# getanteon/alaz

Measured on AMD Instinct MI355X. Metric: L7 edge-events/s ingested->scored service-map, higher is better.
Workload: dtype u64; 1 GPU; C3 device-resident replay: 10000 pods / 5000 services / 1000000 edges, 10000000 HTTP l7 events per window already in HBM, 2-layer SAGE + MLP score, partitioned K1 (variant 0, 8-byte records, 512 partitions); 2-batch HBM ring (value excludes PCIe: see end_to_end with --full); events_per_window=10000000, layers=2, windows_in_flight=1, parallelism=1 GPU

## Files before the change

### alaz_amd/csrc/servicegraph.hip

```cpp
#include <hip/hip_runtime.h>
#include <hip/hip_ext.h>

#include <algorithm>
#include <cmath>
#include <cstdio>
#include <cstring>
#include <chrono>
#include <condition_variable>
#include <thread>
#include <mutex>
#include <string>
#include <unordered_map>
#include <vector>

#include <dlfcn.h>

#include "join_host.hpp"
#include "sg_plan.hpp"
#include "sg_kernels.h"
#include "sg_sel.h"
#include "sg_trend.h"
#include "sg_node_trend.h"
#include "sg_rank.h"
#include "shard_seq.hpp"
// ... 367 lines not shown
    for (u32 k = 0; k < l; k++) n += 2 * (size_t)(k == 0 ? SG_F_IN : SG_F_HID) * SG_F_HID + SG_F_HID;
    return n;
}

void launch_halo_lists(sg_engine* e, hipStream_t s, u32* req, u32 capp) {
    if (e->plan.k6_one_wg) {
        if (e->d.ncap <= K6_FLAGS_LDS) hipLaunchKernelGGL(k6_halo_build_padded<true>, dim3(1), dim3(1024), 0, s, e->d, req, capp);
        else hipLaunchKernelGGL(k6_halo_build_padded<false>, dim3(1), dim3(1024), 0, s, e->d, req, capp);
        return;
    }
    hipLaunchKernelGGL(k6_halo_lists, dim3(((size_t)e->d.ncap + 1023) / 1024), dim3(1024), 0, s, e->d, req, capp, ++e->k6_epoch, 1u);
}
int do_close(sg_engine* e, hipStream_t s, const u32* d_union, const u32* d_union_n, u32 ob_mode = 1, u32 stride = 0, u32 gworld = 0, bool fuse_in = false) {
    int rc = sync_tables(e, s);
    if (rc) return rc;
    Dev dloc = e->d;
    if (dloc.warm && (size_t)e->cur < e->note_seen.size()) {
        volatile u64* note = e->h_note[e->cur];
        const u64 seq = note[0];
        if (seq != e->note_seen[e->cur]) {
            e->note_seen[e->cur] = seq;
            const u64 v = note[1];
            const u32 cold = (u32)(v & 0xFFu); const bool obip = (v & 0x100ull) != 0;
            e->cold_streak = cold == 2 ? e->cold_streak + 1 : 0;
            e->obip_streak = (cold == 1 && obip) ? e->obip_streak + 1 : 0;
            if (e->cold_streak >= 3) { e->plain_left = 32; e->cold_streak = 0; }
            if (e->obip_streak >= 4) { e->plain_left = 64; e->obip_streak = 0; }
        }
    }
    if (dloc.warm && e->plain_left) { e->plain_left--; dloc.warm = 0; }
    if ((size_t)e->cur < e->plain_slot.size()) e->plain_slot[e->cur] = e->d.warm && !dloc.warm;
    const Dev& d = dloc;
    bool warm_try = d.warm && e->warm_on;
    const u32 wt = warm_try ? 1u : 0u;
    {
        Timed tp(e, s, 2);
        if (ob_mode == 1) hipLaunchKernelGGL(kc_prepare, dim3(1), dim3(1024), 0, s, d, (u64)e->n_known, (u64)e->n_labels_decl, e->d_ob_list, (const u32*)e->d_ob_n, e->plan.ob_list_cap, 1u, (const u32*)nullptr, 0u, 0u, wt);
        else if (ob_mode == 0) hipLaunchKernelGGL(kc_prepare, dim3(1), dim3(1024), 0, s, d, (u64)e->n_known, (u64)e->n_labels_decl, const_cast<u32*>(d_union), d_union_n, e->plan.ob_list_cap, 0u, (const u32*)nullptr, 0u, 0u, wt);
        else hipLaunchKernelGGL(kc_prepare, dim3(1), dim3(1024), 0, s, d, (u64)e->n_known, (u64)e->n_labels_decl, e->d_ob_list, (const u32*)e->d_ob_n, e->plan.ob_list_cap, 2u, d_union, stride, gworld, wt);
    }
    if (d.variant == 0) {
        const bool tk = ((e->timing >> 7) & 1u) && e->closes % e->timing_stride == 0;
        hipEvent_t ta = tk ? get_event(e) : nullptr, tb = tk ? get_event(e) : nullptr;
        Dev db = d; db.batch_state = e->window_events_in == 0 ? 2u : 0u;
        db.kept_compact = d.warm;
        const dim3 grid(d.narrow ? d.npb : d.np), block(e->plan.k1b_threads);
        if (d.warm && warm_try) {
            hipExtLaunchKernelGGL(e->fn.k1b_try, grid, block, (uint32_t)e->plan.k1b_lds, s, ta, tb, 0u, db);
            if (tk) { TimingRec r; r.a = ta; r.b = tb; r.kernel = 7; e->trecs.push_back(r); ta = get_event(e); tb = get_event(e); }
        }
        hipExtLaunchKernelGGL(d.warm ? e->fn.k1b_cold : e->fn.k1b, grid, block, (uint32_t)e->plan.k1b_lds, s, ta, tb, 0u, db);
        if (tk) { TimingRec r; r.a = ta; r.b = tb; r.kernel = 7; e->trecs.push_back(r); }
    }
    {
        Timed t(e, s, 2);
        Dev dk = d;
        dk.kept_compact = d.warm;
        if (d.warm) {
            dk.rowptr = d.k_rowptr; dk.col = d.k_col; dk.csr_from = d.k_from; dk.acc_csr = d.k_acc; dk.max_edges = (u64)d.npb * d.pcap;
            dk.st_sum = e->scr_sum[e->cur]; dk.st_max = e->scr_max[e->cur]; dk.row_mu = e->scr_mu[e->cur]; dk.row_sd = e->scr_mu[e->cur] + d.ncap + 1;
        }
        if (d.variant == 1) {
            const u32 ntiles = e->plan.ecap / K2_TILE;
            hipLaunchKernelGGL(k2_edge_count, dim3(ntiles), dim3(256), 0, s, d);
            hipLaunchKernelGGL(k2_scan_tiles, dim3(1), dim3(1024), 0, s, d, ntiles);
            hipLaunchKernelGGL(k2_edge_compact, dim3(ntiles), dim3(256), 0, s, d);
        }
        if (d.dh_g) hipLaunchKernelGGL(k2_deg_hist, dim3(d.dh_g), dim3(K2_DH_THREADS), ((size_t)d.ncap + 1) * sizeof(u32), s, dk);
        const size_t rpr = d.dh_g ? K2_RP_ROWS_DH : K2_RP_ROWS;
        hipLaunchKernelGGL(e->fn.k2_rowptr, dim3(((size_t)d.ncap + rpr) / rpr), dim3(1024), 0, s, dk, ++e->rp_epoch);
        if (d.variant == 1) hipLaunchKernelGGL(k2_scatter_table, dim3(grid_for(e->cfg.max_edges, 256)), dim3(256), 0, s, d);
        else hipLaunchKernelGGL(k2_scatter_parts, dim3(d.npb), dim3(256), 0, s, dk);
        hipLaunchKernelGGL(k2_rowsort_gather, dim3(std::max(2, std::min(4096, 2 * K2_LONG_WGS + grid_for(d.ncap, 8)))), dim3(256), 2 * (size_t)d.k2_sortw * sizeof(u32), s, dk);
        if (d.warm) {
            const unsigned kg = (unsigned)(((u64)d.npb * d.pcap + KW_CH - 1) / KW_CH) + KW_CAPW;
            hipLaunchKernelGGL(kw_compact, dim3(kg), dim3(KW_THREADS), (size_t)KW_ROWS * 5 * sizeof(u64), s, d, ++e->kw_epoch, dk.st_sum, dk.st_max, (u64)(e->closes + 1), e->slots.size() > 1 ? 1u : 0u);
        }
    }
    {
        Timed t3(e, s, 8);
        const u32 fin = d.warm ? (u32)std::min<u64>(64, ((u64)d.ncap + 255) / 256) : 1u;
        if (fuse_in && e->plan.k3_fuse_allowed) {
            const u32 finp = d.warm ? (fin + 3) / 4 : 1u;
            hipLaunchKernelGGL(k3_in_part, dim3(e->plan.k3_ranges * e->plan.k3_slices + finp), dim3(1024), e->plan.k3in_lds, s, d, e->plan.k3_slices, finp);
            e->in_fused_slices = e->plan.k3_slices;
        } else {
            hipLaunchKernelGGL(k3_in_part, dim3(e->plan.k3_ranges * e->plan.k3_slices), dim3(1024), e->plan.k3in_lds, s, d, e->plan.k3_slices, 0u);
            hipLaunchKernelGGL(k3_in_reduce, dim3(grid_for((u64)d.ncap * 6, 256, 1024) + fin), dim3(256), 0, s, d, e->plan.k3_slices, fin);
            e->in_fused_slices = 0;
        }
    }
    HIP_TRY(e, hipGetLastError());
    e->closed = true;
    e->window_events_in = 0;
    e->closes++;
    return SG_OK;
}

int do_features(sg_engine* e, hipStream_t s) {
    const Dev& d = e->d;
    Timed t(e, s, 3);
    const int nbn = grid_for(d.ncap, 128), nbe = grid_for(e->cfg.max_edges, 256, 4096);
    hipLaunchKernelGGL(k3_node_features, dim3(nbn + nbe), dim3(256), 0, s, d, (u32)nbn, e->in_fused_slices);
    e->in_fused_slices = 0;
    HIP_TRY(e, hipGetLastError());
    return SG_OK;
}

int note_w_read(sg_engine* e, hipStream_t s) {
    for (auto& r : e->w_readers) if (r.first == s) { HIP_TRY(e, hipEventRecord(r.second, s)); return SG_OK; }
    for (size_t i = 0; i < e->w_readers.size();) {
        if (hipEventQuery(e->w_readers[i].second) == hipSuccess) { hipEventDestroy(e->w_readers[i].second); e->w_readers[i] = e->w_readers.back(); e->w_readers.pop_back(); }
        else i++;
    }
    hipEvent_t v = nullptr;
    HIP_TRY(e, hipEventCreateWithFlags(&v, hipEventDisableTiming));
    e->w_readers.emplace_back(s, v);
    HIP_TRY(e, hipEventRecord(v, s));
    return SG_OK;
}

int do_layer(sg_engine* e, u32 l, hipStream_t s, bool fuse_proj) {
    const Dev& d = e->d;
    if (!e->have_w) { e->err = "sg_load_weights not called"; return SG_ESTATE; }
    const float* Wl = e->d_W + layer_offset(l);
    const float* Wh = e->d_W + layer_offset(e->cfg.layers);
    const int grid = grid_for(d.ncap, 16);
    const bool pj = fuse_proj && l + 1 == e->cfg.layers && d.world == 1;
    Timed t(e, s, 4);
    const bool split = e->plan.k4_split;
    const int wide = l != 0;
    const float* hin = wide ? d.h[l] : d.x0;
    if (split) hipLaunchKernelGGL(kK4Gather[wide], dim3(grid_for(d.ncap, K4G_ROWS, 4096 * 8 / K4G_ROWS)), dim3(K4G_ROWS * 64), 0, s, d, hin);
    hipLaunchKernelGGL(e->fn.k4_layer[wide][pj], dim3(grid), dim3(k4_threads(wide ? 64 : 32, pj, split)), 0, s, d, hin, d.h[l + 1], Wl, Wh);
    HIP_TRY(e, hipGetLastError());
    return fuse_proj ? SG_OK : note_w_read(e, s);
}

static_assert(sizeof(sg_edge_vanished) == 64 && sgplan::kTrendThreads == K8_THREADS && sgplan::kTrendMaxWgs <= K8_SCAN_THREADS,
              "plan_trend / plan_vanished size the launches of sg_trend.h");
template <class Row>
TrendArgs baseline_args(const sg_engine* e, const sg_engine::Baseline<Row>& t) {
    const sg_trend_params& p = t.p;
    TrendArgs a{};
    a.ctr = e->d.ctr; a.ob_sorted = e->d.ob_sorted; a.max_obip = e->d.max_obip;
    a.cap = t.plan.entries;
    a.buf[0] = t.buf[0]; a.buf[1] = t.buf[1];
    a.th = t.th; a.blk = t.blk; a.ctl = t.ctl;
    a.w = t.w + 1; a.warmup = p.warmup; a.ttl = p.ttl;
    a.alpha = std::ldexp(1.0, -(int)p.shift); a.lat_floor = (double)p.lat_floor_ns; a.err_floor = (double)p.err_floor;
    return a;
}
template <class Row, class F>
int enqueue_baseline(sg_engine* e, sg_engine::Baseline<Row>& t, hipStream_t s, F launch) {
    if (t.pending) HIP_TRY(e, hipStreamWaitEvent(s, t.ev, 0));
    launch();
    HIP_TRY(e, hipGetLastError());
    HIP_TRY(e, hipEventRecord(t.ev, s));
    t.pending = true;
    t.w++;
    return SG_OK;
}
int launch_trend(sg_engine* e, hipStream_t s) {
    sg_engine::Baseline<sg_edge_trend>& t = e->trend;
    TrendArgs a = baseline_args(e, t);
    a.rows = e->d.rows; a.max_edges = e->cfg.max_edges; a.out = t.rows[e->cur];
    sg_engine::Vanished& v = e->vanished;
    return enqueue_baseline(e, t, s, [&] {
        if (v.on) {
            VanArgs va{};
            va.out = v.rows[e->cur]; va.count = v.count[e->cur]; va.th = v.th; va.blk = v.blk;
            va.max_rows = v.plan.rows; va.silent = v.p.silent_windows; va.min_seen = v.p.min_seen;
            hipLaunchKernelGGL(k8_count_v, dim3(t.plan.wgs), dim3(K8_THREADS), 0, s, a, va);
            hipLaunchKernelGGL(k8_scan_v, dim3(1), dim3(K8_SCAN_THREADS), 0, s, a, t.plan.wgs, va);
            hipLaunchKernelGGL(k8_write_v, dim3(t.plan.wgs), dim3(K8_THREADS), 0, s, a, va);
            v.valid[e->cur] = 1;
        } else {
            hipLaunchKernelGGL(k8_count, dim3(t.plan.wgs), dim3(K8_THREADS), 0, s, a);
            hipLaunchKernelGGL(k8_scan, dim3(1), dim3(K8_SCAN_THREADS), 0, s, a, t.plan.wgs);
            hipLaunchKernelGGL(k8_write, dim3(t.plan.wgs), dim3(K8_THREADS), 0, s, a);
        }
    });
}
static_assert(sgplan::kNodesThreads == K9_THREADS && sgplan::kNodesChunk == K9_CHUNK && sgplan::kNodesRangeNodes == K9_IN_NR &&
              sgplan::kNodesMaxWgs == K9_MAX_WGS && sgplan::kNodesMaxWgs <= K9_SCAN_THREADS && sgplan::kNodesSideBytes == sizeof(K9Side),
              "plan_nodes sizes the launches of sg_nodes.h");
// ... 1844 lines not shown
```

### alaz_amd/csrc/sg_k3.h

```cpp
#pragma once

__device__ __forceinline__ void alive_mark(const Dev& d, u32 g, u32 G, u32 t) {
    const u64 n_all = d.ctr[C_ALIVE_N];
    if (n_all == 0) return;
    const u32 n = (u32)(n_all < d.alive_cap ? n_all : d.alive_cap);
    const u32 nk = (u32)d.ctr[C_N_KNOWN], nl = (u32)d.ctr[C_N_LABELS], nob = (u32)d.ctr[C_N_OBIP];
    for (u32 i = g * 1024 + t; i < n; i += G * 1024) {
        const u64 key = d.alive_keys[i];
        const u32 f = dense_of(d, (u32)(key >> 32), nk, nl, nob), to = dense_of(d, (u32)key, nk, nl, nob);
        bool ok = f != SG_NONE && to != SG_NONE;
        if (ok) {
            u32 lo = d.rowptr[f], hi = d.rowptr[f + 1];
            if ((u64)hi > d.max_edges) hi = (u32)d.max_edges;
            const u32 end = hi;
            while (lo < hi) { const u32 m = (lo + hi) >> 1; if (d.col[m] < to) lo = m + 1; else hi = m; }
            ok = lo < end && d.col[lo] == to;
            if (ok) {
                atomicAdd(&d.alive_csr[lo], 1u);
                atomicAdd(&d.st_sum[(size_t)f * SG_NODE_STAT_SUM_WORDS + ST_OUT_ALIVE], 1ull);
                atomicAdd(&d.st_sum[(size_t)to * SG_NODE_STAT_SUM_WORDS + ST_IN_ALIVE], 1ull);
            }
        }
        if (!ok) atomicAdd(&d.ctr[C_ALIVE_DROP], 1ull);
    }
}

__global__ __launch_bounds__(1024) void k3_in_part(Dev d, u32 S, u32 fin) {
    extern __shared__ __attribute__((aligned(16))) unsigned char smem[];
    const u32 E = (u32)d.ctr[C_N_EDGES], N = (u32)d.ctr[C_N_NODES];
    const u32 G = gridDim.x - fin, g = blockIdx.x, t = threadIdx.x;
    if (g >= G) {
        if (d.warm) kw_finish_rows(d, (g - G) * 1024 + t, fin * 1024);
        else if (g == gridDim.x - 1) k2_split_finish(d, t, 1024);
        return;
    }
    SG_STAMP(d, 3, 0);
    if (g == 0 && t == 0 && d.warm && !d.ctr[C_COLD] && d.ctr[C_DELTA_N]) {
        d.ctr[C_KEPT_E] += (u64)d.dc_rowptr[d.max_known + d.max_labels];
        d.ctr[C_KEPT_BUF] ^= 1ull;
    }
    alive_mark(d, g, G, t);
    const u32 r = g / S, sl = g % S, n0 = r * K3_IN_NR;
    if (n0 >= N) return;
    const u32 nr = N - n0 < K3_IN_NR ? N - n0 : K3_IN_NR;
    u64* acc = reinterpret_cast<u64*>(smem);
    for (u32 i = t; i < nr * 6; i += 1024) acc[i] = 0;
    __syncthreads();
    SG_STAMP(d, 3, 1);
    const u32 per = (E + S - 1) / S, p0 = sl * per < E ? sl * per : E, p1 = p0 + per < E ? p0 + per : E;
    constexpr int K3Q = 8;
    u32 nxt[K3Q];
#pragma unroll
    for (int q = 0; q < K3Q; q++) { const u32 p = p0 + t + q * 1024; nxt[q] = p < p1 ? d.col[p] - n0 : 0xFFFFFFFFu; }
    for (u32 pb = p0 + t; pb < p1; pb += 1024 * K3Q) {
        u32 to[K3Q];
        ulonglong2 x[K3Q], y[K3Q];
#pragma unroll
        for (int q = 0; q < K3Q; q++) {
            to[q] = nxt[q];
            if (to[q] < nr) { const ulonglong2* a = reinterpret_cast<const ulonglong2*>(d.acc_csr + (size_t)(pb + q * 1024) * 4); x[q] = a[0]; y[q] = a[1]; }
        }
#pragma unroll
        for (int q = 0; q < K3Q; q++) { const u32 p = pb + 1024 * K3Q + q * 1024; nxt[q] = p < p1 ? d.col[p] - n0 : 0xFFFFFFFFu; }
#pragma unroll
        for (int q = 0; q < K3Q; q++) if (to[q] < nr) {
            u64* o = acc + (size_t)to[q] * 6;
            atomicAdd(&o[0], 1ull); atomicAdd(&o[1], x[q].x & 0xFFFFFFFFull); if (x[q].x >> 32) atomicAdd(&o[2], x[q].x >> 32);
            atomicAdd(&o[3], x[q].y); atomicAdd(&o[4], y[q].y); atomicMax(&o[5], y[q].x);
        }
    }
    SG_STAMP(d, 3, 2);
    __syncthreads();
    SG_STAMP(d, 3, 3);
    u64* out = d.in_part + ((size_t)r * S + sl) * K3_IN_NR * 6;
    for (u32 i = t; i < nr * 6; i += 1024) out[i] = acc[i];
    SG_STAMP(d, 3, 4);
}
__global__ __launch_bounds__(256) void k3_in_reduce(Dev d, u32 S, u32 fin) {
    const u32 N = (u32)d.ctr[C_N_NODES];
    if (blockIdx.x >= gridDim.x - fin) {
        if (d.warm) kw_finish_rows(d, (blockIdx.x - (gridDim.x - fin)) * 256 + threadIdx.x, fin * 256);
        else if (blockIdx.x == gridDim.x - 1) k2_split_finish(d, threadIdx.x, 256);
        return;
    }
    const u32 GW = gridDim.x - fin;
    for (u64 i = (u64)blockIdx.x * 256 + threadIdx.x; i < (u64)N * 6; i += (u64)GW * 256) {
        const u32 v = (u32)(i / 6), k = (u32)(i % 6), r = v / K3_IN_NR;
        const u64* p = d.in_part + ((size_t)r * S * K3_IN_NR + (v - r * K3_IN_NR)) * 6 + k;
        const size_t st = (size_t)K3_IN_NR * 6;
        u64 a = 0;
        u32 sl = 0;
        if (k == 5) {
            for (; sl + 8 <= S; sl += 8) {
                u64 x[8];
#pragma unroll
                for (int q = 0; q < 8; q++) x[q] = p[(size_t)(sl + q) * st];
#pragma unroll
                for (int q = 0; q < 8; q++) a = x[q] > a ? x[q] : a;
            }
            for (; sl < S; sl++) { const u64 x = p[(size_t)sl * st]; a = x > a ? x : a; }
            d.st_max[(size_t)v * 2 + 1] = a;
        } else {
            for (; sl + 8 <= S; sl += 8) {
                u64 x[8];
#pragma unroll
                for (int q = 0; q < 8; q++) x[q] = p[(size_t)(sl + q) * st];
#pragma unroll
                for (int q = 0; q < 8; q++) a += x[q];
            }
            for (; sl < S; sl++) a += p[(size_t)sl * st];
            d.st_sum[(size_t)v * SG_NODE_STAT_SUM_WORDS + (k == 0 ? ST_IN_DEG : k == 1 ? ST_IN_CNT : k == 2 ? ST_IN_ERR : k == 3 ? ST_IN_SUM : ST_IN_SSQ)] = a;
        }
    }
}

__global__ __launch_bounds__(256) void k3_node_features(Dev d, u32 nb_nodes, u32 S_in) {
    if (blockIdx.x >= nb_nodes) {
        const u32 E = (u32)d.ctr[C_N_EDGES];
        for (u32 p = (blockIdx.x - nb_nodes) * 256 + threadIdx.x; p < E; p += (gridDim.x - nb_nodes) * 256) edge_features(d, p);
        return;
    }
    const u32 N = (u32)d.ctr[C_N_NODES], nk = (u32)d.ctr[C_N_KNOWN];
    const u32 side = threadIdx.x & 1u;
    for (u32 v0 = blockIdx.x * 128; v0 < N; v0 += nb_nodes * 128) {
        const u32 v = v0 + (threadIdx.x >> 1);
        const bool live = v < N;
        float a[7] = {0.0f, 0.0f, 0.0f, 0.0f, 0.0f, 0.0f, 0.0f};
        if (live) {
            u64* s = d.st_sum + (size_t)v * SG_NODE_STAT_SUM_WORDS;
            u64 dg, c, er, sm, sq, mx;
            if (S_in && side) {
                const u32 r = v / K3_IN_NR;
                const ulonglong2* p = reinterpret_cast<const ulonglong2*>(d.in_part + ((size_t)r * S_in * K3_IN_NR + (v - r * K3_IN_NR)) * 6);
                const size_t st = (size_t)K3_IN_NR * 3;
                dg = c = er = sm = sq = mx = 0;
                u32 sl = 0;
                for (; sl + 4 <= S_in; sl += 4) {
                    ulonglong2 x[4][3];
#pragma unroll
                    for (int q = 0; q < 4; q++) { x[q][0] = p[(size_t)(sl + q) * st]; x[q][1] = p[(size_t)(sl + q) * st + 1]; x[q][2] = p[(size_t)(sl + q) * st + 2]; }
#pragma unroll
                    for (int q = 0; q < 4; q++) { dg += x[q][0].x; c += x[q][0].y; er += x[q][1].x; sm += x[q][1].y; sq += x[q][2].x; mx = x[q][2].y > mx ? x[q][2].y : mx; }
                }
                for (; sl < S_in; sl++) {
                    const ulonglong2 a0 = p[(size_t)sl * st], a1 = p[(size_t)sl * st + 1], a2 = p[(size_t)sl * st + 2];
                    dg += a0.x; c += a0.y; er += a1.x; sm += a1.y; sq += a2.x; mx = a2.y > mx ? a2.y : mx;
                }
                s[ST_IN_DEG] = dg; s[ST_IN_CNT] = c; s[ST_IN_ERR] = er; s[ST_IN_SUM] = sm; s[ST_IN_SSQ] = sq; d.st_max[(size_t)v * 2 + 1] = mx;
            } else {
                dg = s[ST_OUT_DEG + side]; c = s[ST_OUT_CNT + side]; er = s[ST_OUT_ERR + side]; sm = s[ST_OUT_SUM + side]; sq = s[ST_OUT_SSQ + side];
                mx = d.st_max[(size_t)v * 2 + side];
            }
            a[0] = (float)log1p((double)dg);
            a[1] = (float)log1p((double)c);
            a[2] = (float)log1p(mean_us(sm, c) / 1000.0);
            a[3] = c ? (float)((double)er / (double)c) : 0.0f;
            a[4] = (float)log1p((double)mx / 1e6);
            a[5] = (float)log1p(std_us(sm, sq, c) / 1000.0);
            a[6] = (float)log1p((double)s[ST_OUT_ALIVE + side]);
        }
        float b[7];
#pragma unroll
        for (int k = 0; k < 7; k++) b[k] = __shfl_xor(a[k], 1, 64);
        if (!live) continue;
        float4* o = reinterpret_cast<float4*>(d.x0 + (size_t)v * SG_F_IN);
        if (side == 0) {
            const u32 kind = v < nk ? d.kind[v] : 0u;
            o[0] = make_float4(a[0], b[0], a[1], b[1]);
            o[1] = make_float4(a[2], b[2], a[3], b[3]);
            o[2] = make_float4(a[4], b[4], kind == SG_NODE_POD ? 1.0f : 0.0f, kind == SG_NODE_SERVICE ? 1.0f : 0.0f);
            o[3] = make_float4(kind == 0 ? 1.0f : 0.0f, a[5], b[5], 1.0f);
        } else {
            o[4] = make_float4(b[6], a[6], 0.0f, 0.0f);
#pragma unroll
            for (int q = 5; q < (int)SG_F_IN / 4; q++) o[q] = make_float4(0.0f, 0.0f, 0.0f, 0.0f);
        }
    }
    if (blockIdx.x == 0 && threadIdx.x == 0) {
        const u64 n = d.ctr[C_ALIVE_N];
        d.ctr[C_ALIVE_SEEN] = n;
        d.ctr[C_ALIVE_DROPPED] = d.ctr[C_ALIVE_DROP] + (n > d.alive_cap ? n - d.alive_cap : 0);
        d.ctr[C_ALIVE_N] = 0; d.ctr[C_ALIVE_DROP] = 0;
    }
}

__global__ __launch_bounds__(256) void k_reset_window(Dev d) {
    const u64 tid = (u64)blockIdx.x * 256 + threadIdx.x, nt = (u64)gridDim.x * 256;
    const u64 nc = (u64)d.ncap + 1;
    if (!d.dh_g) for (u64 i = tid; i < nc * SG_DEG_REP; i += nt) { d.deg[i * SG_DEG_STRIDE] = 0; if (d.warm) d.deg2[i * SG_DEG_STRIDE] = 0; }
    for (u64 i = tid; i < nc; i += nt) d.cursor[i] = 0;
    for (u64 i = tid; i < (u64)d.ncap * SG_NODE_STAT_SUM_WORDS; i += nt) d.st_sum[i] = 0;
    for (u64 i = tid; i < (u64)d.ncap * SG_NODE_STAT_MAX_WORDS; i += nt) d.st_max[i] = 0;
    for (u64 i = tid; i <= d.obmask; i += nt) d.obkeys[i] = 0;
    for (u64 i = tid; i < (u64)SG_MAX_K1_WGS * WS_WORDS; i += nt) d.wgstat[i] = (i % WS_WORDS) == WS_TMIN ? ~0ull : 0ull;
    if (tid == 0) { d.ctr[C_OVF_N] = 0; d.ctr[C_ALIVE_N] = 0; d.ctr[C_ALIVE_DROP] = 0; }
    if (d.variant == 1 && d.ctr[C_EDGES_FOUND] > d.max_edges) {
        for (u64 i = tid; i <= d.emask; i += nt) {
            d.ekeys[i] = SG_EKEY_EMPTY;
            ulonglong2* a = reinterpret_cast<ulonglong2*>(d.eacc + (size_t)i * 4);
            a[0] = make_ulonglong2(0, 0); a[1] = make_ulonglong2(0, 0);
            if (d.hist) { uint4* hs = reinterpret_cast<uint4*>(d.hist_src + (size_t)i * SG_HIST_BINS); const uint4 z = make_uint4(0, 0, 0, 0); hs[0] = z; hs[1] = z; hs[2] = z; hs[3] = z; }
        }
    }
}
```

### alaz_amd/csrc/sg_plan.hpp

```cpp
#pragma once
#include <algorithm>
#include <array>
#include <cmath>
#include <cstdint>
#include <cstdlib>
#include <cstring>
#include <optional>
#include <string>

#include "../../include/servicegraph.h"
#include "sg_sizes.h"

namespace sgplan {

typedef uint32_t u32;
typedef uint64_t u64;

constexpr size_t kLdsBytes = 160 * 1024;
constexpr int kStageSlots = 32;

inline u32 next_pow2(u64 v) { u64 p = 1; while (p < v) p <<= 1; return (u32)p; }
inline int grid_for(u64 items, int per_block, int cap = 2048) {
    u64 g = (items + per_block - 1) / per_block;
    return (int)std::max<u64>(1, std::min<u64>(g, (u64)cap));
}

struct DeviceFacts {
    int cus = 256;
    size_t lds_bytes = kLdsBytes;
};

struct Overrides {
    typedef std::optional<std::string> Knob;
    Knob ablate, np, ht, ct, nwg, nsub, split, warm, k1a, k1_narrow, k1_legacy, k1b_u, k1b_threads, k1b_pack, k1b_no_order,
         l2_global, l2_u32, dh_g, k3_slices, k3_no_fuse, k4_fused, k5_grid, k6_one_wg, dense_valu, copy_streams, stage_slots, arena;
};
struct KnobName { const char* name; Overrides::Knob Overrides::*field; };
constexpr KnobName kKnobs[] = {
    {"SG_ABLATE", &Overrides::ablate}, {"SG_NP", &Overrides::np}, {"SG_HT", &Overrides::ht}, {"SG_CT", &Overrides::ct},
    {"SG_NWG", &Overrides::nwg}, {"SG_NSUB", &Overrides::nsub}, {"SG_SPLIT", &Overrides::split}, {"SG_WARM", &Overrides::warm},
    {"SG_K1A", &Overrides::k1a}, {"SG_K1_NARROW", &Overrides::k1_narrow}, {"SG_K1_LEGACY", &Overrides::k1_legacy},
    {"SG_K1B_U", &Overrides::k1b_u}, {"SG_K1B_THREADS", &Overrides::k1b_threads}, {"SG_K1B_PACK", &Overrides::k1b_pack},
    {"SG_K1B_NO_ORDER", &Overrides::k1b_no_order}, {"SG_L2_GLOBAL", &Overrides::l2_global}, {"SG_L2_U32", &Overrides::l2_u32},
    {"SG_DH_G", &Overrides::dh_g}, {"SG_K3_SLICES", &Overrides::k3_slices}, {"SG_K3_NO_FUSE", &Overrides::k3_no_fuse},
    {"SG_K4_FUSED", &Overrides::k4_fused}, {"SG_K5_GRID", &Overrides::k5_grid}, {"SG_K6_ONE_WG", &Overrides::k6_one_wg},
    {"SG_DENSE_VALU", &Overrides::dense_valu}, {"SG_COPY_STREAMS", &Overrides::copy_streams}, {"SG_STAGE_SLOTS", &Overrides::stage_slots},
    {"SG_ARENA", &Overrides::arena},
};
#ifdef SG_DEV_KNOBS
inline Overrides from_env() {
    Overrides o;
    for (const KnobName& k : kKnobs) if (const char* v = std::getenv(k.name)) o.*k.field = std::string(v);
    return o;
}
#endif
inline int ival(const Overrides::Knob& k) { return std::atoi(k->c_str()); }
inline u64 uval(const Overrides::Knob& k) { return std::strtoull(k->c_str(), nullptr, 0); }

struct Plan {
    u32 variant = 0, narrow = 0, hist = 0, agg_slots = 3, nb = 0, np = 0, pb = 0, nwg = 256, k1b_split = 1, k1b_ht = 0, npb = 0, rb = 0,
        pcap = 0, sa = 0, sn = 0, sw = 0, punits = 0, ss = 0, pslots = 0, ovf_cap = 0, warm = 0;
    u32 k1b_threads = 1024, k1b_u = 4;
    bool k1b_pack = false;
    bool k1b_order = false;
    size_t k1b_lds = 0;
    u32 ecap = 0, obcap = 0, ob_list_cap = 0, ncap = 0, max_obip = 1, alive_cap = 0, hub_cap = 0, max_blocks = 0;
    u64 kept_edges = 0;
    u32 max_known = 0;
    u32 k3_ranges = 1, k3_slices = 8;
    size_t k3in_lds = 0;
    u32 k2_sortw = 0, dh_g = 0, dh_ppw = 0, dh_ns = 0;
    bool k4_split = false;
    u32 k5_grid = 0;
    bool k3_fuse_allowed = true;
    bool k6_one_wg = false;
    bool use_mfma = true;
    u32 cus = 1;
    int k1_grid = 0, n_copy = 1, n_stage = 16;
    bool arena_on = false;
    u32 n_slots = 1;
    u32 ablate = 0;
};

struct PassA {
    bool l2_u16 = false, k1a_team = false, l2_in_lds = false;
    u32 k1a_nsub = 2, k1a_teams = 2, k1a_nt = 1024, k1a_ct = 2048;
    size_t k1a_lds = 0;
};

inline int check_config(const sg_config& in, sg_config* out) {
    constexpr uint32_t kCfgMin = 88;
    if (in.struct_size < kCfgMin || in.struct_size > 4096) return SG_EINVAL;
    sg_config c; std::memset(&c, 0, sizeof c);
    std::memcpy(&c, &in, std::min<size_t>(in.struct_size, sizeof c));
    c.struct_size = (uint32_t)sizeof c;
    if (c.abi_version != SG_ABI_VERSION || c.layers < 1 || c.layers > SG_MAX_LAYERS || c.max_edges == 0 ||
        c.max_known_nodes == 0 || c.world == 0 || c.rank >= c.world || c.max_known_nodes > 0x3FFFFFFFu)
        return SG_EINVAL;
    if (c.max_batch == 0) c.max_batch = 1u << 20;
    if (c.max_ips == 0) c.max_ips = c.max_known_nodes;
    if (c.max_window_events == 0) c.max_window_events = c.max_batch;
    *out = c;
    return SG_OK;
}

inline int make_plan(const sg_config& cfg, const DeviceFacts& dev, const Overrides& ov, Plan* out, std::string* why) {
    sg_config chk;
    if (check_config(cfg, &chk) != SG_OK) { if (why) *why = "invalid config"; return SG_EINVAL; }
    Plan p;
    const size_t lds = dev.lds_bytes;
    if (ov.arena) p.arena_on = ival(ov.arena) != 0;
    p.k1_grid = std::min<int>(SG_MAX_K1_WGS, dev.cus * 8);
    p.cus = (u32)std::max(1, dev.cus);
    p.use_mfma = !(ov.dense_valu && (*ov.dense_valu)[0] == '1');
    p.max_known = cfg.max_known_nodes;

    const u64 ME = cfg.max_edges;
    p.ecap = next_pow2(std::max<u64>(2 * ME, K2_TILE));
    p.obcap = next_pow2(std::max<u64>(2 * (u64)cfg.max_outbound_ips, 64));
    p.ob_list_cap = next_pow2(std::max<u64>((u64)cfg.max_outbound_ips * std::max<u32>(cfg.world, 1), 64));
    p.max_obip = std::max<u32>(cfg.max_outbound_ips, 1);
    p.ncap = cfg.max_known_nodes + cfg.max_labels + p.max_obip;

    p.variant = cfg.k1_variant == 1 ? 1u : 0u;
    p.hist = (cfg.flags & SG_CFG_EDGE_HISTOGRAM) ? 1u : 0u;
    p.agg_slots = p.hist ? 5u : 3u;
    const u64 cn = (u64)cfg.max_known_nodes + cfg.max_labels + p.obcap;
    u32 nb = 12; while ((1ull << nb) < cn && nb < 31) nb++;
    bool narrow = p.variant == 0 && !p.hist && cfg.k1_variant != 2 && !ov.k1_legacy && nb <= 24;
    const bool small_window = ME < (1ull << 18) && cfg.max_window_events <= (2ull << 20);
    if (cfg.k1_variant == 0 && small_window && !ov.k1_narrow) narrow = false;
    u64 np = 0;
    if (narrow) {
        np = next_pow2(std::max<u64>((ME + 2699) / 2700, 256));
        u32 pbt = 0; while ((1ull << pbt) < np) pbt++;
        if (np > 2048 || 2 * nb - pbt > 31) narrow = false;
    }
    p.k1b_split = 1;
    if (narrow) {
        if (ME / np > 1150) { p.k1b_split = 2; p.k1b_ht = 2048; }
        else p.k1b_ht = ME / np > 550 ? 2048 : 1024;
        if (ov.split) { const int x = ival(ov.split); if (x == 1 || x == 2) { p.k1b_split = (u32)x; p.k1b_ht = ME / (np * x) > 1150 ? 4096 : (ME / (np * x) > 550 ? 2048 : 1024); } }
    } else {
        np = next_pow2(std::max<u64>((ME + 1249) / 1250, 256));
        if (np > 4096) np = 4096;
        if (cfg.k1_variant != 1 && ME > (u64)4096 * 1400) p.variant = 1;
        p.k1b_ht = ME / np > 600 ? 2048 : 1024;
        if (p.hist && p.k1b_ht == 2048) { p.k1b_ht = 1024; np = std::min<u64>(4096, np * 2); }
    }
    p.np = (u32)np; p.nwg = 256;
    if (ov.np) { const u64 x = uval(ov.np); if (x >= 64 && x <= (narrow ? 2048u : 4096u) && (x & (x - 1)) == 0) p.np = (u32)x; }
    if (ov.ht) { const u64 x = uval(ov.ht); if (x >= 256 && x <= (narrow ? 4096u : 2048u) && (x & (x - 1)) == 0) p.k1b_ht = (u32)x; }
    if (ov.nwg) { const u64 x = uval(ov.nwg); if (x >= 1 && x <= (u64)SG_MAX_K1_WGS) p.nwg = (u32)x; }
    p.pb = 0; while ((1u << p.pb) < p.np) p.pb++;
    if (narrow && 2 * nb - p.pb > 31) { p.np = (u32)np; p.pb = 0; while ((1u << p.pb) < p.np) p.pb++; }
    p.narrow = (narrow && p.variant == 0) ? 1u : 0u;
    if (!p.narrow) p.k1b_split = 1;
    p.warm = (p.narrow && !p.hist && !(cfg.flags & SG_CFG_NO_WARM) && ((cfg.flags & SG_CFG_WARM) || ME >= (1ull << 18))) ? 1u : 0u;
    if (ov.warm) p.warm = (ival(ov.warm) != 0 && p.narrow && !p.hist) ? 1u : 0u;
    p.npb = p.np * p.k1b_split;
    p.nb = nb; p.rb = 2 * nb - p.pb;
    p.pcap = p.narrow ? p.k1b_ht * 13 / 16 : p.k1b_ht * 3 / 4;
    const double m = (double)cfg.max_window_events / ((double)p.np * p.nwg);
    p.sa = std::min<u32>(24, std::max<u32>(8, (2 * 2048 / p.np + 6 + 1) & ~1u));
    if (p.narrow) {
        p.sn = ((u32)(2.0 * m + 8.0 * std::sqrt(m + 1.0) + 24.0) + 1u) & ~1u;
        p.sn = std::min<u32>(p.sn, (1u << 20) - 16);
        p.sw = std::min<u32>(64, std::max<u32>(8, p.sn / 8));
        p.punits = (p.sn + 2 * p.sw + 5 * p.sa + 15) / 16 * 16;
        p.sn = p.punits - 2 * p.sw - 5 * p.sa;
        p.ss = 0; p.pslots = 0;
    } else {
        p.ss = (u32)(2.0 * m + 8.0 * std::sqrt(m + 1.0) + 24.0);
        p.ss = (p.ss + p.agg_slots * p.sa + 7) / 8 * 8 - p.agg_slots * p.sa;
        p.ss = std::min<u32>(p.ss, (1u << 20) - 8);
        p.pslots = p.ss + p.agg_slots * p.sa;
    }
    p.ovf_cap = 1u << 16;
    p.k1b_threads = 1024u;
    if (p.variant == 0)
        p.k1b_lds = p.narrow ? ((size_t)p.k1b_ht * 36 + 8 + (size_t)p.k1b_ht / 4 + 12 + 15) / 16 * 16 : (size_t)p.k1b_ht * (8 + 32 + (p.hist ? 4 * SG_HIST_BINS : 0));
    if (p.narrow) p.k1b_u = 2 * p.k1b_lds > lds && m > 24.0 ? 8 : 4;
    if (ov.k1b_u) { if (ival(ov.k1b_u) == 8) p.k1b_u = 8; if (ival(ov.k1b_u) == 4) p.k1b_u = 4; }
    if (p.k1b_u == 8) p.warm = 0;
    p.k1b_pack = p.narrow && (u64)p.sn * p.nwg < 65536ull;
    if (ov.k1b_pack) { if (ival(ov.k1b_pack) == 0) p.k1b_pack = false; }
    if (ov.k1b_threads) { const u64 x = uval(ov.k1b_threads); if ((x == 256 && !p.narrow) || x == 512 || x == 1024) p.k1b_threads = (u32)x; }
    if (p.narrow && p.k1b_ht / p.k1b_threads > 4) p.k1b_threads = 1024u;
    p.k1b_order = p.narrow && !ov.k1b_no_order;
    p.max_blocks = p.variant == 0 ? (u32)std::min<u64>(1024, std::max<u64>(64, (u64)cfg.max_ips / 32)) : 2u;
    if (p.variant == 0) p.ecap = K2_TILE;
    p.alive_cap = cfg.max_alive ? cfg.max_alive : 65536u;
    p.kept_edges = p.warm ? std::max<u64>(ME, (u64)p.npb * p.pcap) : ME;
    p.hub_cap = (u32)std::min<u64>(p.kept_edges / 256 + 16, 1u << 24);

    p.k3_ranges = (p.ncap + K3_IN_NR - 1) / K3_IN_NR;
    p.k3_slices = (u32)std::min<u64>((u64)p.k3_ranges * K3_IN_SMAX <= p.cus ? K3_IN_SMAX : 32, std::max<u64>(8, ME / 8192));
    if (ov.k3_slices) { const u64 x = uval(ov.k3_slices); if (x >= 1 && x <= 256) p.k3_slices = (u32)x; }
    p.k3in_lds = (size_t)K3_IN_NR * 48;
    {
        const u64 bw = ((u64)p.ncap + 31) / 32;
        p.k2_sortw = bw <= K2_SORT_LDS ? K2_SORT_LDS : (u32)std::min<u64>(K2_SORT_LDS_MAX, (bw + 255) / 256 * 256);
    }
    {
        u32 g = std::min<u32>(K2_DH_GMAX, p.variant == 0 ? p.npb : 0u);
        if (ME < (1ull << 19)) g = 0;
        if (p.warm) g = 0;
        else if (ov.dh_g) { const u64 x = uval(ov.dh_g); g = (x >= 16 && x <= K2_DH_GMAX && (x & (x - 1)) == 0 && p.variant == 0 && x <= p.npb) ? (u32)x : 0u; }
        if (g >= 16 && (g & (g - 1)) == 0 && p.npb % g == 0 && ((size_t)p.ncap + 1) * sizeof(u32) <= 128u * 1024u && (u64)p.npb * p.pcap < (1ull << 32)) {
            p.dh_g = g; p.dh_ppw = p.npb / g; p.dh_ns = (p.ncap + 1 + 63u) & ~63u;
        }
    }
    p.ablate = ov.ablate ? (u32)std::strtoul(ov.ablate->c_str(), nullptr, 0) : 0u;
    p.k4_split = cfg.max_edges > (1u << 17);
    if (ov.k4_fused) p.k4_split = ival(ov.k4_fused) == 0;
    p.k5_grid = (u32)grid_for(cfg.max_edges, 32, 3 * (int)p.cus);
    if (ov.k5_grid) { const int x = ival(ov.k5_grid); if (x >= 1 && x <= 65535) p.k5_grid = (u32)std::min(grid_for(cfg.max_edges, 32, 65535), x); }
    p.k3_fuse_allowed = !ov.k3_no_fuse;
    p.k6_one_wg = (bool)ov.k6_one_wg;
    if (ov.copy_streams) p.n_copy = ival(ov.copy_streams) == 2 ? 2 : 1;
    if (ov.stage_slots) p.n_stage = std::min(kStageSlots, std::max(2, ival(ov.stage_slots)));
    p.n_slots = std::min<u32>(std::max<u32>(cfg.windows_in_flight, 1), 8);
    *out = p;
    return SG_OK;
}

inline bool plan_pass_a(const Plan& p, uint32_t l1_entries, size_t l2_bytes, const Overrides& ov, PassA* out) {
    PassA a;
    const size_t lds_cap = kLdsBytes;
    const size_t l1b = (size_t)l1_entries * 8, l2b = l2_bytes;
    const size_t stage_max = (size_t)K1A_NJ * K1A_THREADS * 16;
    if (p.narrow) {
        a.l2_u16 = p.max_known <= 16384 && !ov.l2_u32;
        const size_t l2lds = a.l2_u16 ? l2b / 2 : l2b;
        if (ov.nsub) { const int x = ival(ov.nsub); if (x == 1 || x == 2) a.k1a_nsub = (u32)x; }
        const bool want_tile = ov.k1a && *ov.k1a == "tile", force_team = ov.k1a && *ov.k1a == "team";
        const size_t fixed_tile = (size_t)p.np * 24 + 64 + (size_t)K1T_TS(a.k1a_nsub) * 8 + l1b;
        const int teams = 2, nt = 1024;
        const size_t stage_team = (size_t)K1A_NJ * nt * 16;
        const bool team_ok = (p.np == 256 || p.np == 512 || p.np == 1024) && (size_t)p.np * p.nwg * p.punits * 8 < ((size_t)1 << 31) && l1b <= stage_team;
        a.k1a_teams = (u32)teams; a.k1a_nt = (u32)nt;
        const size_t fixed_team = K1M_LDS_FIXED(p.np, teams, nt) + l1b;
        auto pick = [&](size_t fixed, u32 ct_min, size_t stage_cap, u32& ct, bool& in_lds) {
            ct = 0; in_lds = false;
            for (u32 c : {1024u, 512u, 256u, 128u}) if (c >= ct_min && (size_t)c * 40 + fixed + l2lds <= lds_cap && l1b + l2b <= stage_cap) { in_lds = true; ct = c; break; }
            if (!ct) for (u32 c : {1024u, 512u, 256u, 128u, 64u}) if (c >= ct_min && (size_t)c * 40 + fixed <= lds_cap) { ct = c; break; }
        };
        u32 ct = 0; bool in_lds = false;
        if (!want_tile && team_ok) { pick(fixed_team, force_team ? 64u : 256u, stage_team, ct, in_lds); a.k1a_team = ct != 0; }
        if (!ct) pick(fixed_tile, 64u, stage_max, ct, in_lds);
        const size_t fixed = a.k1a_team ? fixed_team : fixed_tile;
        a.l2_in_lds = in_lds;
        if (ov.l2_global) a.l2_in_lds = false;
        if (ov.ct) { const u32 x = (u32)std::strtoul(ov.ct->c_str(), nullptr, 0); if (x >= 64 && x <= 2048 && (x & (x - 1)) == 0 && (size_t)x * 40 + fixed + (a.l2_in_lds ? l2lds : 0) <= lds_cap) ct = x; }
        if (!ct || l1b > stage_max) return false;
        a.k1a_ct = ct;
        a.k1a_lds = (size_t)ct * 40 + fixed + (a.l2_in_lds ? l2lds : 0);
        *out = a;
        return true;
    }
    const size_t fixed = (size_t)p.np * 4 + 64 + l1b;
    const size_t slot = p.hist ? 72 : 40;
    u32 ct = 0;
    for (u32 c : {2048u, 1024u, 512u}) if ((size_t)c * slot + fixed + l2b <= lds_cap && l1b + l2b <= stage_max) { a.l2_in_lds = true; ct = c; break; }
    if (!ct) for (u32 c : {2048u, 1024u, 512u, 256u, 128u, 64u}) if ((size_t)c * slot + fixed <= lds_cap) { ct = c; break; }
    if (ov.ct) { const u32 x = (u32)std::strtoul(ov.ct->c_str(), nullptr, 0); if (x >= 64 && x <= 2048 && (x & (x - 1)) == 0 && (size_t)x * slot + fixed + (a.l2_in_lds ? l2b : 0) <= lds_cap) ct = x; }
    if (ov.l2_global) a.l2_in_lds = false;
    if (!ct || l1b > stage_max) return false;
    a.k1a_ct = ct;
    a.k1a_lds = (size_t)ct * slot + fixed + (a.l2_in_lds ? l2b : 0);
    *out = a;
    return true;
}

enum K1aFamily { K1A_GLOBAL = 0, K1A_WIDE = 1, K1A_TILE = 2, K1A_TEAM = 3 };
enum K1bFamily { K1B_NONE = 0, K1B_MERGE = 1, K1B_STREAM = 2 };
constexpr int kK1bWarmU = 2;
struct PassAKernel {
    int family = K1A_GLOBAL;
// ... 274 lines not shown
```

### alaz_amd/csrc/sg_sizes.h

```cpp
#pragma once

#define SG_MAX_K1_WGS 2048

#define K1A_THREADS 1024
#define K1A_NJ      6
#define K1T_THREADS 1024
#define K1T_CHUNK   4096u
#define K1T_TS(NSUB) (K1T_CHUNK * (NSUB))
#define K1M_LDS_FIXED(np, teams, nt) ((size_t)(np) * 4 * (2 + 4 * (teams)) + 128 + ((size_t)(nt) * 4 + 4) * 8)

#define K2_TILE 2048
#define K2_DH_GMAX 128
#define K2_SORT_LDS 4096
#define K2_SORT_LDS_MAX 16384

#define K3_IN_NR    3072
#define K3_IN_SMAX  48

#define KW_ROWS 512
```

Baseline: 23.03 billion events/s.

## Interleave node-to-range mapping in k3 in-degree partial reduction

Result: no change. 23.23 billion events/s (median of 6 runs) (+0.9%).

```diff
diff --git a/alaz_amd/csrc/servicegraph.hip b/alaz_amd/csrc/servicegraph.hip
--- a/alaz_amd/csrc/servicegraph.hip
+++ b/alaz_amd/csrc/servicegraph.hip
@@ -473,11 +473,11 @@
         const u32 fin = d.warm ? (u32)std::min<u64>(64, ((u64)d.ncap + 255) / 256) : 1u;
         if (fuse_in && e->plan.k3_fuse_allowed) {
             const u32 finp = d.warm ? (fin + 3) / 4 : 1u;
-            hipLaunchKernelGGL(k3_in_part, dim3(e->plan.k3_ranges * e->plan.k3_slices + finp), dim3(1024), e->plan.k3in_lds, s, d, e->plan.k3_slices, finp);
+            hipLaunchKernelGGL(k3_in_part, dim3(e->plan.k3_ranges * e->plan.k3_slices + finp), dim3(1024), e->plan.k3in_lds, s, d, e->plan.k3_slices, finp, e->plan.k3_map);
             e->in_fused_slices = e->plan.k3_slices;
         } else {
-            hipLaunchKernelGGL(k3_in_part, dim3(e->plan.k3_ranges * e->plan.k3_slices), dim3(1024), e->plan.k3in_lds, s, d, e->plan.k3_slices, 0u);
-            hipLaunchKernelGGL(k3_in_reduce, dim3(grid_for((u64)d.ncap * 6, 256, 1024) + fin), dim3(256), 0, s, d, e->plan.k3_slices, fin);
+            hipLaunchKernelGGL(k3_in_part, dim3(e->plan.k3_ranges * e->plan.k3_slices), dim3(1024), e->plan.k3in_lds, s, d, e->plan.k3_slices, 0u, e->plan.k3_map);
+            hipLaunchKernelGGL(k3_in_reduce, dim3(grid_for((u64)d.ncap * 6, 256, 1024) + fin), dim3(256), 0, s, d, e->plan.k3_slices, fin, e->plan.k3_map);
             e->in_fused_slices = 0;
         }
     }
@@ -492,7 +492,7 @@
     const Dev& d = e->d;
     Timed t(e, s, 3);
     const int nbn = grid_for(d.ncap, 128), nbe = grid_for(e->cfg.max_edges, 256, 4096);
-    hipLaunchKernelGGL(k3_node_features, dim3(nbn + nbe), dim3(256), 0, s, d, (u32)nbn, e->in_fused_slices);
+    hipLaunchKernelGGL(k3_node_features, dim3(nbn + nbe), dim3(256), 0, s, d, (u32)nbn, e->in_fused_slices, e->plan.k3_map);
     e->in_fused_slices = 0;
     HIP_TRY(e, hipGetLastError());
     return SG_OK;
diff --git a/alaz_amd/csrc/sg_k3.h b/alaz_amd/csrc/sg_k3.h
--- a/alaz_amd/csrc/sg_k3.h
+++ b/alaz_amd/csrc/sg_k3.h
@@ -25,9 +25,9 @@
     }
 }
 
-__global__ __launch_bounds__(1024) void k3_in_part(Dev d, u32 S, u32 fin) {
+__global__ __launch_bounds__(1024) void k3_in_part(Dev d, u32 S, u32 fin, K3InMap m) {
     extern __shared__ __attribute__((aligned(16))) unsigned char smem[];
-    const u32 E = (u32)d.ctr[C_N_EDGES], N = (u32)d.ctr[C_N_NODES];
+    const u32 E = (u32)d.ctr[C_N_EDGES];
     const u32 G = gridDim.x - fin, g = blockIdx.x, t = threadIdx.x;
     if (g >= G) {
         if (d.warm) kw_finish_rows(d, (g - G) * 1024 + t, fin * 1024);
@@ -40,9 +40,11 @@
         d.ctr[C_KEPT_BUF] ^= 1ull;
     }
     alive_mark(d, g, G, t);
-    const u32 r = g / S, sl = g % S, n0 = r * K3_IN_NR;
-    if (n0 >= N) return;
-    const u32 nr = N - n0 < K3_IN_NR ? N - n0 : K3_IN_NR;
+    const u32 r = g / S, sl = g % S, R = m.R;
+    const u64 ncov = (u64)R * K3_IN_NR, nn = d.ctr[C_N_NODES];
+    const u32 N = (u32)(nn < ncov ? nn : ncov);
+    if (r >= N) return;
+    const u32 nr = k3_in_idx(m, N - 1 - r) + 1;
     u64* acc = reinterpret_cast<u64*>(smem);
     for (u32 i = t; i < nr * 6; i += 1024) acc[i] = 0;
     __syncthreads();
@@ -51,20 +53,21 @@
     constexpr int K3Q = 8;
     u32 nxt[K3Q];
 #pragma unroll
-    for (int q = 0; q < K3Q; q++) { const u32 p = p0 + t + q * 1024; nxt[q] = p < p1 ? d.col[p] - n0 : 0xFFFFFFFFu; }
+    for (int q = 0; q < K3Q; q++) { const u32 p = p0 + t + q * 1024; nxt[q] = p < p1 ? d.col[p] : 0xFFFFFFFFu; }
     for (u32 pb = p0 + t; pb < p1; pb += 1024 * K3Q) {
-        u32 to[K3Q];
+        u32 ix[K3Q];
         ulonglong2 x[K3Q], y[K3Q];
 #pragma unroll
         for (int q = 0; q < K3Q; q++) {
-            to[q] = nxt[q];
-            if (to[q] < nr) { const ulonglong2* a = reinterpret_cast<const ulonglong2*>(d.acc_csr + (size_t)(pb + q * 1024) * 4); x[q] = a[0]; y[q] = a[1]; }
-        }
-#pragma unroll
-        for (int q = 0; q < K3Q; q++) { const u32 p = pb + 1024 * K3Q + q * 1024; nxt[q] = p < p1 ? d.col[p] - n0 : 0xFFFFFFFFu; }
-#pragma unroll
-        for (int q = 0; q < K3Q; q++) if (to[q] < nr) {
-            u64* o = acc + (size_t)to[q] * 6;
+            const u32 to = nxt[q], i = k3_in_idx(m, to);
+            ix[q] = to < N && to - i * R == r ? i : 0xFFFFFFFFu;
+            if (ix[q] != 0xFFFFFFFFu) { const ulonglong2* a = reinterpret_cast<const ulonglong2*>(d.acc_csr + (size_t)(pb + q * 1024) * 4); x[q] = a[0]; y[q] = a[1]; }
+        }
+#pragma unroll
+        for (int q = 0; q < K3Q; q++) { const u32 p = pb + 1024 * K3Q + q * 1024; nxt[q] = p < p1 ? d.col[p] : 0xFFFFFFFFu; }
+#pragma unroll
+        for (int q = 0; q < K3Q; q++) if (ix[q] != 0xFFFFFFFFu) {
+            u64* o = acc + (size_t)ix[q] * 6;
             atomicAdd(&o[0], 1ull); atomicAdd(&o[1], x[q].x & 0xFFFFFFFFull); if (x[q].x >> 32) atomicAdd(&o[2], x[q].x >> 32);
             atomicAdd(&o[3], x[q].y); atomicAdd(&o[4], y[q].y); atomicMax(&o[5], y[q].x);
         }
@@ -76,7 +79,7 @@
     for (u32 i = t; i < nr * 6; i += 1024) out[i] = acc[i];
     SG_STAMP(d, 3, 4);
 }
-__global__ __launch_bounds__(256) void k3_in_reduce(Dev d, u32 S, u32 fin) {
+__global__ __launch_bounds__(256) void k3_in_reduce(Dev d, u32 S, u32 fin, K3InMap m) {
     const u32 N = (u32)d.ctr[C_N_NODES];
     if (blockIdx.x >= gridDim.x - fin) {
         if (d.warm) kw_finish_rows(d, (blockIdx.x - (gridDim.x - fin)) * 256 + threadIdx.x, fin * 256);
@@ -85,8 +88,9 @@
     }
     const u32 GW = gridDim.x - fin;
     for (u64 i = (u64)blockIdx.x * 256 + threadIdx.x; i < (u64)N * 6; i += (u64)GW * 256) {
-        const u32 v = (u32)(i / 6), k = (u32)(i % 6), r = v / K3_IN_NR;
-        const u64* p = d.in_part + ((size_t)r * S * K3_IN_NR + (v - r * K3_IN_NR)) * 6 + k;
+        const u32 v = (u32)(i / 6), k = (u32)(i % 6), ix = k3_in_idx(m, v), r = v - ix * m.R;
+        if (ix >= K3_IN_NR) continue;
+        const u64* p = d.in_part + ((size_t)r * S * K3_IN_NR + ix) * 6 + k;
         const size_t st = (size_t)K3_IN_NR * 6;
         u64 a = 0;
         u32 sl = 0;
@@ -114,7 +118,7 @@
     }
 }
 
-__global__ __launch_bounds__(256) void k3_node_features(Dev d, u32 nb_nodes, u32 S_in) {
+__global__ __launch_bounds__(256) void k3_node_features(Dev d, u32 nb_nodes, u32 S_in, K3InMap m) {
     if (blockIdx.x >= nb_nodes) {
         const u32 E = (u32)d.ctr[C_N_EDGES];
         for (u32 p = (blockIdx.x - nb_nodes) * 256 + threadIdx.x; p < E; p += (gridDim.x - nb_nodes) * 256) edge_features(d, p);
@@ -130,8 +134,8 @@
             u64* s = d.st_sum + (size_t)v * SG_NODE_STAT_SUM_WORDS;
             u64 dg, c, er, sm, sq, mx;
             if (S_in && side) {
-                const u32 r = v / K3_IN_NR;
-                const ulonglong2* p = reinterpret_cast<const ulonglong2*>(d.in_part + ((size_t)r * S_in * K3_IN_NR + (v - r * K3_IN_NR)) * 6);
+                const u32 ix = k3_in_idx(m, v), r = v - ix * m.R;
+                const ulonglong2* p = reinterpret_cast<const ulonglong2*>(d.in_part + ((size_t)r * S_in * K3_IN_NR + ix) * 6);
                 const size_t st = (size_t)K3_IN_NR * 3;
                 dg = c = er = sm = sq = mx = 0;
                 u32 sl = 0;
diff --git a/alaz_amd/csrc/sg_plan.hpp b/alaz_amd/csrc/sg_plan.hpp
--- a/alaz_amd/csrc/sg_plan.hpp
+++ b/alaz_amd/csrc/sg_plan.hpp
@@ -68,6 +68,7 @@
     u64 kept_edges = 0;
     u32 max_known = 0;
     u32 k3_ranges = 1, k3_slices = 8;
+    K3InMap k3_map = {1, 1u << 31, 31};
     size_t k3in_lds = 0;
     u32 k2_sortw = 0, dh_g = 0, dh_ppw = 0, dh_ns = 0;
     bool k4_split = false;
@@ -87,6 +88,13 @@
     u32 k1a_nsub = 2, k1a_teams = 2, k1a_nt = 1024, k1a_ct = 2048;
     size_t k1a_lds = 0;
 };
+
+inline K3InMap k3_in_map(u32 ranges) {
+    const u32 R = std::max<u32>(ranges, 1);
+    u32 l = 0; while ((1ull << l) < R) l++;
+    const u32 sh = 31 + l;
+    return K3InMap{R, (u32)(((1ull << sh) + R - 1) / R), sh};
+}
 
 inline int check_config(const sg_config& in, sg_config* out) {
     constexpr uint32_t kCfgMin = 88;
@@ -195,6 +203,7 @@
     p.hub_cap = (u32)std::min<u64>(p.kept_edges / 256 + 16, 1u << 24);
 
     p.k3_ranges = (p.ncap + K3_IN_NR - 1) / K3_IN_NR;
+    p.k3_map = k3_in_map(p.k3_ranges);
     p.k3_slices = (u32)std::min<u64>((u64)p.k3_ranges * K3_IN_SMAX <= p.cus ? K3_IN_SMAX : 32, std::max<u64>(8, ME / 8192));
     if (ov.k3_slices) { const u64 x = uval(ov.k3_slices); if (x >= 1 && x <= 256) p.k3_slices = (u32)x; }
     p.k3in_lds = (size_t)K3_IN_NR * 48;
diff --git a/alaz_amd/csrc/sg_sizes.h b/alaz_amd/csrc/sg_sizes.h
--- a/alaz_amd/csrc/sg_sizes.h
+++ b/alaz_amd/csrc/sg_sizes.h
@@ -16,5 +16,10 @@
 
 #define K3_IN_NR    3072
 #define K3_IN_SMAX  48
+struct K3InMap { unsigned R, mul, sh; };
+#ifdef __HIPCC__
+__host__ __device__
+#endif
+inline unsigned k3_in_idx(const K3InMap& m, unsigned v) { return (unsigned)(((unsigned long long)v * m.mul) >> m.sh); }
 
 #define KW_ROWS 512
```
